# jonassibbesen/rpvg

Measured on AMD Instinct MI355X. Metric: read-pairs quantified/sec, higher is better.
Workload: dtype f64

## Files before the change

### include/rpvg_hip.h

```cpp
#ifndef RPVG_HIP_H
#define RPVG_HIP_H

#include <stdint.h>

#include "rpvg_batch.h"
#include "rpvg_rows.h"
#include "rpvg_index.h"
#include "rpvg_table.h"
#include "rpvg_samples.h"

#ifdef __cplusplus
extern "C" {
#endif

typedef enum rpvg_hip_status {
    RPVG_HIP_OK = 0,
    RPVG_HIP_ERR_NO_DEVICE = -1,
    RPVG_HIP_ERR_RUNTIME = -2,
    RPVG_HIP_ERR_INVALID = -3,
    RPVG_HIP_ERR_ALLOC = -4,
    RPVG_HIP_ERR_UNSUPPORTED = -5
} rpvg_hip_status;

typedef struct rpvg_hip_ctx rpvg_hip_ctx;
// ... 302 lines not shown
void rpvg_hip_gibbs_samples_free(rpvg_hip_ctx * ctx, rpvg_hip_gibbs_samples * samples);
int rpvg_hip_gibbs_table_build_resident(rpvg_hip_ctx * ctx, const rpvg_hip_gibbs_samples * samples, const rpvg_hip_em_problems * problems,
                                        uint32_t num_clusters, const uint64_t * cluster_path_off, const double * total_count,
                                        uint32_t num_gibbs_samples, rpvg_hip_gibbs_table ** table_out);

#define RPVG_HIP_COMM_ID_BYTES 128
int rpvg_hip_comm_unique_id(uint8_t * id_out);
int rpvg_hip_comm_init(rpvg_hip_ctx * ctx, const uint8_t * id, int world_size, int rank);
int rpvg_hip_comm_destroy(rpvg_hip_ctx * ctx);
int rpvg_hip_comm_init_all(rpvg_hip_ctx * const * ctxs, int num_contexts);
int rpvg_hip_comm_allreduce_sum_f64(rpvg_hip_ctx * ctx, double * device_buf, uint64_t n);
int rpvg_hip_gather(rpvg_hip_ctx * ctx, const double * local_values, uint64_t local_count, const uint64_t * counts, double * all_values);

int rpvg_hip_synth_dense_cluster(rpvg_hip_ctx * ctx, uint64_t seed, uint64_t num_rows, uint32_t num_paths,
                                 double * device_matrix, uint64_t ld, double * device_counts);
int rpvg_hip_synth_dense_rows(rpvg_hip_ctx * ctx, uint64_t seed, uint64_t row_begin, uint64_t num_rows, uint32_t num_paths,
                              double * device_matrix, uint64_t ld, double * device_counts);

int rpvg_hip_synth_dense_cluster_batch(rpvg_hip_ctx * ctx, uint64_t seed, uint64_t num_rows, uint32_t num_paths,
                                       rpvg_hip_batch ** batch_out);

int rpvg_hip_debug_log(rpvg_hip_ctx * ctx, uint64_t n, const double * x, double * out, int32_t use_table);

#define RPVG_HIP_EM_KERNELS 12
typedef struct rpvg_hip_em_kernel_stats {
    double ms;
    uint64_t launches;
    uint64_t problems;
    uint64_t iterations;
    uint64_t max_iterations;
    double alg_bytes;
} rpvg_hip_em_kernel_stats;
const char * rpvg_hip_em_kernel_name(int index);

typedef struct rpvg_hip_kernel_stats {
    double em_sparse_ms;      uint64_t em_sparse_launches;   double em_sparse_alg_bytes;
    double em_dense_ms;       uint64_t em_dense_launches;    double em_dense_alg_bytes;
    double loglik_ms;         uint64_t loglik_launches;      double loglik_evals;
    double build_ms;          uint64_t build_launches;
    double h2d_ms;            double h2d_bytes;
    uint64_t em_iterations_total;
    double search_pairs_possible; double search_pairs_table; double search_pairs_kept;
    rpvg_hip_em_kernel_stats em_kernel[RPVG_HIP_EM_KERNELS];
    double collapse_ms;
    double busy_ms;
    double gibbs_ms;
    double search_tile_ms;    uint64_t search_tile_launches;
    uint64_t gibbs_calls_completed;
    uint64_t gibbs_count_grid_problems;
    uint64_t gibbs_count_grid_iterations;
    uint64_t cover_grid_problems;
    uint64_t cover_grid_rounds;
    uint64_t nested_full_calls;
    uint64_t nested_full_sets;
    uint64_t nested_full_retained;
} rpvg_hip_kernel_stats;

int rpvg_hip_stats_get(rpvg_hip_ctx * ctx, rpvg_hip_kernel_stats * stats_out);
int rpvg_hip_stats_reset(rpvg_hip_ctx * ctx);
int rpvg_hip_stats_intervals(rpvg_hip_ctx * ctx, uint64_t capacity, double * start_ms, double * stop_ms, int32_t * family,
                             uint64_t * count_out);

#ifdef __cplusplus
}
#endif

// ... 2 lines not shown
```

### rpvg_amd/csrc/common.hpp

```cpp
#ifndef RPVG_HIP_COMMON_HPP
#define RPVG_HIP_COMMON_HPP

#include <hip/hip_runtime.h>

#include <algorithm>
#include <chrono>
#include <cstdarg>
#include <cstdint>
#include <cstdio>
#include <cstdlib>
#include <cstring>
#include <memory>
#include <mutex>
#include <new>
#include <string>
#include <functional>
#include <vector>

#include "../../include/rpvg_hip.h"
#include "search_plan.hpp"
#include "em_plan.hpp"
#include "batch_forms.hpp"

namespace rpvg_hip_detail {
// ... 771 lines not shown
    DeviceBuffer<uint32_t> d_prow_off, d_pent_col, d_bucket, d_order, d_seg_rows, d_seg_entries;
    DeviceBuffer<double> d_prow_count, d_prow_noise, d_pent_val, d_zero, d_wide_vectors, d_seg_zero, d_seg_total;
    DeviceBuffer<unsigned long long> d_wide_off;
    DeviceBuffer<unsigned char> d_queues;
    unsigned char * zeroed_queues = nullptr;
    std::shared_ptr<void> collapse;
    DeviceBuffer<double> fused_matrix[kEmMaxFusedDense];
    EmFusedDense fused[kEmMaxFusedDense];
    uint32_t num_fused = 0;
    hipEvent_t filled = nullptr, collapsed = nullptr, collapse_sorted = nullptr;
    EmProblemsView view(const EmProblemList & list, const EmOutputs & out) const {
        EmProblemsView v;
        v.col_off = list.d_col_off;
        v.row_base = list.d_row_base;
        v.ent_base = list.d_ent_base;
        v.kept_rows = out.d_kept_rows;
        v.zero_mass = d_zero.ptr;
        v.total_mass = out.d_total;
        v.prow_off = d_prow_off.ptr;
        v.prow_count = d_prow_count.ptr;
        v.prow_noise = d_prow_noise.ptr;
        v.pent_col = d_pent_col.ptr;
        v.pent_val = d_pent_val.ptr;
        return v;
    }
    ~EmSolveWork() {
        if (filled) (void) hipEventDestroy(filled);
        if (collapsed) (void) hipEventDestroy(collapsed);
        if (collapse_sorted) (void) hipEventDestroy(collapse_sorted);
    }
};
size_t emQueuesBytes();
uint32_t emFillSegmentRows();

struct EmGridControl {
    uint32_t done;
    uint32_t iterations;
    uint32_t conv_its;
    uint32_t viol;
    uint32_t error;
    uint32_t arrived;
};

struct EmGridProblem {
    uint32_t problem, columns;
    uint32_t rows, entries;
    uint32_t merged, pad;
    uint64_t row_base, ent_base, col_begin;
    double total_mass, zero_mass;
};

struct EmGridStorage {
    EmProblemsView problems;
    double * abundances;
    double * noise_count;
    uint32_t * iterations;
    const EmFusedDense * fused = nullptr;
    uint32_t num_fused = 0;
};

uint64_t emGridMinWork();
uint64_t gibbsGridMinWork();
bool emGridDenseRoute(uint32_t columns, uint32_t rows, uint32_t entries);
int runEmGridProblems(rpvg_hip_ctx * ctx, hipStream_t st, const EmGridProblem * problems, uint32_t count, const EmGridStorage & storage,
                      uint32_t max_em_its, double max_rel_em_conv);

// ... 115 lines not shown
```

### rpvg_amd/csrc/em_plan.hpp

```cpp
#ifndef RPVG_EM_PLAN_HPP
#define RPVG_EM_PLAN_HPP

#include <algorithm>
#include <cstddef>
#include <cstdint>

#ifndef RPVG_PLAN_FN
#if defined(__HIPCC__)
#define RPVG_PLAN_FN __host__ __device__ inline
#else
#define RPVG_PLAN_FN inline
#endif
#endif

namespace rpvg_em {

constexpr int kEmBins = 12;
constexpr int kEmGridBin = 11;
constexpr int kEmWideBin = 10;
constexpr int kEmWorkBuckets = 32;
constexpr uint32_t kEmMidGridMax = 8;
constexpr uint32_t kEmMidGridLog2 = 16;
constexpr uint32_t kEmMidBuckets = kEmWorkBuckets - kEmMidGridLog2;
constexpr int kEmStreamedBin = 3;
// ... 37 lines not shown

RPVG_PLAN_FN uint32_t emWorkBucket(const uint32_t rows, const uint32_t entries) {
    uint64_t work = static_cast<uint64_t>(entries) + rows + 1;
    uint32_t lg = 0;
    while (work > 1 && lg < static_cast<uint32_t>(kEmWorkBuckets - 1)) {
        work >>= 1;
        ++lg;
    }
    return static_cast<uint32_t>(kEmWorkBuckets - 1) - lg;
}

RPVG_PLAN_FN bool emIsMidSize(const uint32_t bin, const uint32_t bucket) { return bin == static_cast<uint32_t>(kEmStreamedBin) && bucket < kEmMidBuckets; }
RPVG_PLAN_FN bool emMidGridAllowed(const uint64_t grid_min_work) { return grid_min_work > (1ull << kEmMidGridLog2); }
RPVG_PLAN_FN bool emMidGridMoves(const bool allowed, const uint32_t mid) { return allowed && mid > 0 && mid <= kEmMidGridMax; }
RPVG_PLAN_FN int emRouteOf(const int bin, const uint32_t bucket, const bool moved) {
    return moved && emIsMidSize(static_cast<uint32_t>(bin), bucket) ? kEmGridBin : bin;
}

RPVG_PLAN_FN bool emIsRegisterBin(const int bin) { return bin == 4 || bin == 5 || bin == 6 || bin == 8 || bin == 9; }
RPVG_PLAN_FN int emStatsSlot(const int bin, const bool one_register_launch) {
    return emIsRegisterBin(bin) && one_register_launch ? static_cast<int>(kRegisterKernelIndex) : bin;
}

constexpr int kEmMaxFusedDense = 4;
constexpr uint32_t kEmDenseMaxCols = 2048;
RPVG_PLAN_FN bool emDenseRule(const uint32_t columns, const uint32_t rows, const uint32_t entries) {
    if (columns > kEmDenseMaxCols || columns < 2) return false;
    const uint64_t ld = (static_cast<uint64_t>(columns) + 1) & ~1ull;
    return 8ull * rows * ld <= 12ull * entries + 20ull * rows;
}

constexpr uint32_t kLdsMapPaths = 16384;
constexpr uint32_t kFillSegmentRows = 1024;
constexpr uint64_t kFillLongRowEntries = 32;
constexpr size_t kFillLongRowLds = kFillSegmentRows * (3 * sizeof(uint32_t) + sizeof(double));
constexpr size_t kFillDenseLds = kFillSegmentRows * 2 * sizeof(uint32_t);
constexpr uint64_t kFillLongRowMinWork = 1ull << 18;
RPVG_PLAN_FN size_t emFillDenseLdsBytes(const uint32_t lds_map_paths, const uint64_t widest_ld) {
    return lds_map_paths * sizeof(int32_t) + kFillDenseLds + 4 * static_cast<size_t>(widest_ld) * sizeof(double);
}

struct EmSolveKnobs {
    EmBinRule rule = {1u, 0, 1ull << 18};
    bool no_collapse = false;
    bool no_fused_dense = false;
    bool register_copies = true;
    bool one_register_launch = true;
    bool merged_launches = false;
    bool fill_thread_rows = false;
    double grid_scale = 1.0;
    bool few_streams = false;
    bool launch_early = false;
    bool wait_sort_only = false;
    bool join_on_stream = false;
    bool collapse_debug = false;
    bool has_bound_bytes = false;
    uint64_t bound_bytes = 0;
};

RPVG_PLAN_FN bool emStorageByBound(const uint64_t rows_bound, const uint64_t entries_bound, const uint64_t budget) {
    return rows_bound * 20 + entries_bound * 12 <= budget;
}
template <typename Count>
inline void emStorageBases(const Count * rows, const Count * entries, const uint32_t P, uint64_t * row_base, uint64_t * ent_base, uint64_t * rows_total,
                           uint64_t * entries_total) {
    uint64_t r = 0, e = 0;
    for (uint32_t p = 0; p < P; ++p) {
        row_base[p] = r;
        ent_base[p] = e;
        r += rows[p];
        e += entries[p];
    }
    *rows_total = r;
    *entries_total = e;
}

constexpr size_t kGibbsOneWorkgroupLdsLimit = 160 * 1024;
RPVG_PLAN_FN size_t gibbsOneWorkgroupLds(const uint32_t columns) {
    return (sizeof(double) * (2 * static_cast<size_t>(columns) + 256 / 64 + 2) + 15) & ~static_cast<size_t>(15);
}
RPVG_PLAN_FN bool gibbsTakesGrid(const uint32_t columns, const uint32_t rows, const uint32_t entries, const uint64_t grid_min_work) {
    const bool too_wide = gibbsOneWorkgroupLds(columns) > kGibbsOneWorkgroupLdsLimit;
    const bool too_large = grid_min_work != 0 && static_cast<uint64_t>(rows) + entries >= grid_min_work;
    return too_wide || too_large;
}
RPVG_PLAN_FN bool gibbsGridPossible(const uint32_t max_cols, const uint64_t max_cluster_work, const uint64_t grid_min_work) {
    return gibbsOneWorkgroupLds(max_cols) > kGibbsOneWorkgroupLdsLimit || (grid_min_work != 0 && max_cluster_work >= grid_min_work);
}

struct EmSolveShape {
    uint32_t P = 0, items_bound = 0, max_cols = 0, max_cluster_paths = 0;
    uint64_t max_cluster_work = 0, rows_capacity = 0;
    unsigned long long wide_capacity = 0;
    uint32_t cus = 0;
    int side_streams = 6;
    int hardware_queues = 4;
    bool collapse_wanted = false;
};
constexpr int kEmSideStreams = 6;
constexpr uint32_t kEmCollapseMaxProblems = (1u << 20) - 2;
constexpr uint64_t kEmCollapseMaxRows = 0x7fffffffull;

struct EmFillPlan {
    uint32_t fill_grid = 0;
    uint32_t dense_grid = 0;
    uint32_t lds_map_paths = 0;
    bool long_row_scratch = false;
    size_t fill_lds = 0;
};
inline EmFillPlan planEmFill(const EmSolveShape & s, const EmSolveKnobs & knobs) {
    EmFillPlan f;
    f.fill_grid = std::min<uint32_t>(s.items_bound, s.cus * 8);
    f.dense_grid = std::min<uint32_t>(s.items_bound, s.cus * 4);
    f.lds_map_paths = (std::min<uint32_t>(s.max_cluster_paths, kLdsMapPaths) + 3) & ~3u;
    f.long_row_scratch = !knobs.fill_thread_rows && s.max_cluster_work >= kFillLongRowMinWork;
    f.fill_lds = f.lds_map_paths * sizeof(int32_t) + (f.long_row_scratch ? kFillLongRowLds : 0);
    return f;
}

enum class EmVariant : uint8_t {
    kSparse64Resident, kSparse256Resident, kSparse1024Resident, kSparse256Streamed, kSparse1024Streamed, kSparseWide,
    kRegisterBins,
    kRegister1x16, kRegister2x16, kRegister4x16, kRegister1x32, kRegister2x32,
    kWaveBins,
    kSparse1024Bins
};
constexpr int kEmMainStream = -1;
struct EmLaunch {
    uint32_t bin;
    EmVariant variant;
    uint32_t grid;
    size_t lds;
    int stream;
};
inline bool operator==(const EmLaunch & a, const EmLaunch & b) {
    return a.bin == b.bin && a.variant == b.variant && a.grid == b.grid && a.lds == b.lds && a.stream == b.stream;
}
constexpr int kEmMaxLaunches = 11;

constexpr uint32_t kEmMaxRoles = 6;
struct EmRoles {
    uint32_t variants = 0;
    uint32_t grid = 0;
    uint32_t bin[kEmMaxRoles] = {};
};

struct EmSolvePlan {
    EmFillPlan fill;
    bool collapse = false;
// ... 96 lines not shown
```

### rpvg_amd/csrc/em_sparse.hip

```cpp

#include "common.hpp"

#include "collapse_plan.hpp"
#include "em_block.hpp"

#include <algorithm>
#include <memory>
#include <numeric>

using namespace rpvg_hip_detail;

namespace {

constexpr double kMinEmAbundance = 1e-8;
constexpr uint32_t kMinEmConvIts = 10;
static_assert(kEmBins == RPVG_HIP_EM_KERNELS, "a statistics slot per size bin (em_plan.hpp)");

struct EmQueues {
    uint32_t histogram[kEmBins * kEmWorkBuckets];
    uint32_t bucket_cursor[kEmBins * kEmWorkBuckets];
    uint32_t bin_start[kEmBins];
    uint32_t bin_count[kEmBins];
    uint32_t bin_cursor[kEmBins];
    uint32_t pad;
    unsigned long long wide_cursor;
    unsigned long long wide_overflow;
};


struct FillArgs {
    uint32_t num_problems;
    const uint32_t * num_problems_dev;
    uint32_t num_items;
    const uint32_t * num_items_dev;
    const uint64_t * seg_first;
    const uint32_t * item_problem;
    const uint32_t * prob_cluster;
    const uint32_t * col_path;
    const uint64_t * cluster_row_off;
    const uint64_t * cluster_path_off;
    const uint64_t * row_ent_off;
    const uint32_t * ent_path;
    const double * ent_prob;
    const double * row_count;
    const double * row_noise;
    EmProblemsView problems;
    uint32_t * seg_rows;
    uint32_t * seg_entries;
    double * seg_zero_mass;
    double * seg_total_mass;
    uint32_t * kept_entries;
    uint32_t * prob_bucket;
    EmQueues * queues;
    EmBinRule rule;
    uint32_t lds_map_paths;
    uint32_t long_row_scratch;
    uint32_t num_fused;
    EmFusedDense fused[kEmMaxFusedDense];
};

__device__ inline bool fillLongRows(const FillArgs & args, const uint32_t k) {
    const uint64_t c0 = args.cluster_row_off[k], c1 = args.cluster_row_off[k + 1];
    return args.long_row_scratch && args.row_ent_off[c1] - args.row_ent_off[c0] >= kFillLongRowEntries * (c1 - c0);
}

template <bool WRITE>
__global__ __launch_bounds__(256) void fillSegmentsKernel(const FillArgs args) {
    constexpr int BLOCK = 256;
    extern __shared__ __attribute__((aligned(16))) int32_t lds_map[];
    __shared__ uint32_t scratch[2 * (BLOCK / 64)];
    __shared__ double dscratch[BLOCK / 64];
    const uint32_t num_items = args.num_items_dev ? *args.num_items_dev : args.num_items;
    uint32_t mapped_problem = UINT32_MAX;
    for (uint32_t item = blockIdx.x; item < num_items; item += gridDim.x) {
        const uint32_t p = args.item_problem[item];
        if (WRITE) {
            bool fused = false;
            for (uint32_t f = 0; f < args.num_fused; ++f) fused = fused || args.fused[f].problem == p;
            if (fused) continue;
        }
        const uint32_t segment = static_cast<uint32_t>(item - args.seg_first[p]);
        const uint32_t k = args.prob_cluster[p];
        const uint32_t n_paths = static_cast<uint32_t>(args.cluster_path_off[k + 1] - args.cluster_path_off[k]);
        const uint32_t * cols = args.col_path + args.problems.col_off[p];
        const uint32_t n_cols = args.problems.paths(p);
        const bool use_map = n_paths <= args.lds_map_paths;
        const bool identity = n_cols == n_paths;
        __syncthreads();
        if (use_map && !identity && mapped_problem != p) {
            for (uint32_t i = threadIdx.x; i < n_paths; i += BLOCK) lds_map[i] = -1;
            __syncthreads();
            for (uint32_t c = threadIdx.x; c < n_cols; c += BLOCK) lds_map[cols[c]] = static_cast<int32_t>(c);
            __syncthreads();
            mapped_problem = p;
        }
        auto column_of = [&](const uint32_t path) -> int32_t {
            if (identity) return static_cast<int32_t>(path);
            if (use_map) return lds_map[path];
            uint32_t lo = 0, hi = n_cols;
            while (lo < hi) {
                const uint32_t mid = (lo + hi) >> 1;
                if (cols[mid] < path) lo = mid + 1;
                else hi = mid;
            }
            return (lo < n_cols && cols[lo] == path) ? static_cast<int32_t>(lo) : -1;
        };
        const uint64_t c0 = args.cluster_row_off[k], c1 = args.cluster_row_off[k + 1];
        const uint64_t r0 = c0 + static_cast<uint64_t>(segment) * kFillSegmentRows, r1 = min(c1, r0 + kFillSegmentRows);
        EmProblemsView::Slots at = {};
        if (WRITE) at = args.problems.slots(p);
        uint32_t * off = args.problems.prow_off + at.off;
        uint32_t run_rows = WRITE ? args.seg_rows[item] : 0, run_ent = WRITE ? args.seg_entries[item] : 0;
        double z = 0, t = 0;
        if (fillLongRows(args, k)) {
            uint32_t * row_n = reinterpret_cast<uint32_t *>(lds_map + args.lds_map_paths);
            uint32_t * row_slot = row_n + kFillSegmentRows, * row_eoff = row_slot + kFillSegmentRows;
            double * row_sum = reinterpret_cast<double *>(row_eoff + kFillSegmentRows);
            const uint32_t lane = threadIdx.x & 63, wave = threadIdx.x >> 6;
            const uint32_t seg_n = static_cast<uint32_t>(r1 - r0);
            for (uint32_t i = wave; i < seg_n; i += BLOCK / 64) {
                const uint64_t r = r0 + i;
                const uint64_t e0 = args.row_ent_off[r], e1 = args.row_ent_off[r + 1];
                uint32_t n = 0;
                double sum = 0;
                if (identity) {
                    n = static_cast<uint32_t>(e1 - e0);
                    if (WRITE) {
                        for (uint64_t e = e0 + lane; e < e1; e += 64) sum += args.ent_prob[e];
                    }
                } else {
                    for (uint64_t e = e0 + lane; e < e1; e += 64) {
                        if (column_of(args.ent_path[e]) >= 0) {
                            ++n;
                            sum += args.ent_prob[e];
                        }
                    }
                    for (int d = 32; d >= 1; d >>= 1) n += __shfl_xor(n, d, 64);
                }
                if (WRITE) sum = waveSumF64(sum);
                if (lane == 0) {
                    row_n[i] = n;
                    if (WRITE) row_sum[i] = sum;
                    if (!WRITE) {
                        const double c = args.row_count[r];
                        t += c;
                        if (!n) z += c;
                    }
// ... 28 lines not shown
                    const double nz = args.row_noise[r];
                    if (lane == 0) {
                        off[my_row] = my_ent;
                        args.problems.prow_count[at.row + my_row] = args.row_count[r];
                        args.problems.prow_noise[at.row + my_row] = nz;
                    }
                    const double keep = 1 - nz, rowsum = row_sum[i];
                    const uint64_t e0 = args.row_ent_off[r], e1 = args.row_ent_off[r + 1];
                    uint32_t base = 0;
                    for (uint64_t eb0 = e0; eb0 < e1; eb0 += 64) {
                        const uint64_t e = eb0 + lane;
                        const int32_t c = e < e1 ? column_of(args.ent_path[e]) : -1;
                        const unsigned long long kept = __ballot(c >= 0);
                        if (c >= 0) {
                            const uint32_t to = my_ent + base + static_cast<uint32_t>(__popcll(kept & ((1ull << lane) - 1)));
                            args.problems.pent_col[at.ent + to] = static_cast<uint32_t>(c);
                            args.problems.pent_val[at.ent + to] = (args.ent_prob[e] / rowsum) * keep;
                        }
                        base += static_cast<uint32_t>(__popcll(kept));
                    }
                }
            } else {
                z = blockReduceSum<double, BLOCK>(z, dscratch);
                t = blockReduceSum<double, BLOCK>(t, dscratch);
                if (threadIdx.x == 0) {
                    args.seg_rows[item] = tot_rows;
                    args.seg_entries[item] = tot_ent;
                    args.seg_zero_mass[item] = z;
                    args.seg_total_mass[item] = t;
                }
            }
            continue;
        }
        for (uint64_t rc = r0; rc < r1; rc += BLOCK) {
            const uint64_t r = rc + threadIdx.x;
            uint32_t n = 0;
            double rowsum = 0;
            uint64_t e0 = 0, e1 = 0;
            if (r < r1) {
                e0 = args.row_ent_off[r];
                e1 = args.row_ent_off[r + 1];
                for (uint64_t e = e0; e < e1; ++e) {
                    if (column_of(args.ent_path[e]) >= 0) {
                        ++n;
                        rowsum += args.ent_prob[e];
                    }
                }
                if (!WRITE) {
                    const double c = args.row_count[r];
                    t += c;
                    if (!n) z += c;
                }
            }
            uint32_t slot = n ? 1u : 0u, epos = n, tot_rows, tot_ent;
            blockExclusiveScanPair<BLOCK>(slot, epos, tot_rows, tot_ent, scratch);
            if (WRITE && n) {
                const uint32_t my_row = run_rows + slot;
                uint32_t my_ent = run_ent + epos;
                off[my_row] = my_ent;
                const double nz = args.row_noise[r];
                args.problems.prow_count[at.row + my_row] = args.row_count[r];
                args.problems.prow_noise[at.row + my_row] = nz;
                const double keep = 1 - nz;
                for (uint64_t e = e0; e < e1; ++e) {
                    const int32_t c = column_of(args.ent_path[e]);
                    if (c >= 0) {
                        args.problems.pent_col[at.ent + my_ent] = static_cast<uint32_t>(c);
                        args.problems.pent_val[at.ent + my_ent] = (args.ent_prob[e] / rowsum) * keep;
                        ++my_ent;
                    }
                }
            }
            run_rows += tot_rows;
            run_ent += tot_ent;
        }
        if (!WRITE) {
            z = blockReduceSum<double, BLOCK>(z, dscratch);
            t = blockReduceSum<double, BLOCK>(t, dscratch);
            if (threadIdx.x == 0) {
                args.seg_rows[item] = run_rows;
                args.seg_entries[item] = run_ent;
                args.seg_zero_mass[item] = z;
                args.seg_total_mass[item] = t;
            }
        }
    }
}

template <bool WRITE>
hipError_t launchFillSegments(const FillArgs & fa, const EmFillPlan & plan, hipStream_t st) {
    if (plan.fill_lds > kLdsOptIn) {
        const hipError_t e = hipFuncSetAttribute(reinterpret_cast<const void *>(&fillSegmentsKernel<WRITE>), hipFuncAttributeMaxDynamicSharedMemorySize, static_cast<int>(plan.fill_lds));
        if (e != hipSuccess) return e;
    }
    fillSegmentsKernel<WRITE><<<dim3(plan.fill_grid), dim3(256), plan.fill_lds, st>>>(fa);
    return hipSuccess;
}

constexpr int kDenseRowCache = 32;

__global__ __launch_bounds__(256) void fillDenseRowsKernel(const FillArgs args) {
    constexpr int BLOCK = 256;
// ... 687 lines not shown
    const uint32_t role = blockIdx.x % roles.variants, block = blockIdx.x / roles.variants;
    args.bin = roleBin(roles, role);
    switch (args.bin) {
        case 6: emRegisterBin<4, 16>(args, block, reg_lds); break;
        case 4: emRegisterBin<1, 16>(args, block, reg_lds); break;
        case 5: emRegisterBin<2, 16>(args, block, reg_lds); break;
        case 8: emRegisterBin<1, 32>(args, block, reg_lds); break;
        case 9: emRegisterBin<2, 32>(args, block, reg_lds); break;
        case kWaveSparseBin: emSparseBin<64, true>(args, block, reinterpret_cast<unsigned char *>(reg_lds), nullptr); break;
        default: break;
    }
}

template <int RPL, int COLS>
hipError_t launchEmRegister(const EmLaunchArgs & args, uint32_t grid, size_t lds, hipStream_t stream) {
    if (grid == 0) return hipSuccess;
    emRegisterBinKernel<RPL, COLS><<<dim3(grid), dim3(64), lds, stream>>>(args);
    return hipGetLastError();
}

hipError_t launchEmRegisterBins(const EmLaunchArgs & args, const EmRoles & roles, const size_t lds, hipStream_t stream) {
    const uint32_t grid = roles.variants * roles.grid;
    if (grid == 0) return hipSuccess;
    emRegisterKernel<<<dim3(grid), dim3(64), lds, stream>>>(args, roles);
    return hipGetLastError();
}

}

namespace rpvg_hip_detail {

size_t emQueuesBytes() { return sizeof(EmQueues); }
uint32_t emFillSegmentRows() { return kFillSegmentRows; }

EmSolveKnobs emSolveKnobs() {
    static const EmSolveKnobs once = []() {
        EmSolveKnobs k;
        k.rule.use_register_kernel = RPVG_EXPERIMENT_ENV("RPVG_HIP_NO_REGISTER_EM") == nullptr ? 1u : 0u;
        k.rule.streamed_small_work = RPVG_EXPERIMENT_ENV("RPVG_HIP_EM_STREAM_SMALL") ? std::strtoull(RPVG_EXPERIMENT_ENV("RPVG_HIP_EM_STREAM_SMALL"), nullptr, 10) : 0;
        k.no_collapse = RPVG_EXPERIMENT_ENV("RPVG_HIP_NO_EM_COLLAPSE") != nullptr;
        const char * launches = std::getenv("RPVG_HIP_EM_REGISTER_LAUNCHES");
        k.one_register_launch = !(launches && std::atoi(launches) == 5);
        k.fill_thread_rows = RPVG_EXPERIMENT_ENV("RPVG_HIP_FILL_THREAD_ROWS") != nullptr;
        k.grid_scale = RPVG_EXPERIMENT_ENV("RPVG_HIP_EM_GRID_SCALE") ? std::atof(RPVG_EXPERIMENT_ENV("RPVG_HIP_EM_GRID_SCALE")) : 1.0;
        k.few_streams = RPVG_EXPERIMENT_ENV("RPVG_HIP_EM_FEW_STREAMS") != nullptr;
        k.launch_early = RPVG_EXPERIMENT_ENV("RPVG_HIP_EM_LAUNCH_EARLY") != nullptr;
        k.wait_sort_only = RPVG_EXPERIMENT_ENV("RPVG_HIP_EM_WAIT_SORT_ONLY") != nullptr;
        k.join_on_stream = RPVG_EXPERIMENT_ENV("RPVG_HIP_EM_JOIN_ON_STREAM") != nullptr;
        k.collapse_debug = RPVG_EXPERIMENT_ENV("RPVG_HIP_EM_COLLAPSE_DEBUG") != nullptr;
        return k;
    }();
    EmSolveKnobs k = once;
    k.rule.grid_min_work = emGridMinWork();
    k.no_collapse = k.no_collapse || RPVG_EXPERIMENT_ENV("RPVG_HIP_NO_COLLAPSE") != nullptr;
    k.no_fused_dense = std::getenv("RPVG_HIP_NO_FUSED_DENSE") != nullptr;
    const char * separate = std::getenv("RPVG_HIP_EM_SEPARATE_LAUNCHES");
    k.merged_launches = !(separate && std::atoi(separate) != 0);
    const char * copies = std::getenv("RPVG_HIP_EM_COPIES");
    k.register_copies = copies ? std::atoi(copies) != 0 : true;
    const char * budget = std::getenv("RPVG_HIP_EM_BOUND_BYTES");
    k.has_bound_bytes = budget != nullptr;
    k.bound_bytes = budget ? static_cast<uint64_t>(std::atof(budget)) : 0;
    return k;
}

EmSolveShape emSolveShape(const rpvg_hip_ctx * ctx, const EmProblemList & list, const bool collapse_wanted) {
    EmSolveShape s;
    s.P = list.P_bound;
    s.items_bound = list.items_bound;
    s.max_cols = list.max_cols;
    s.max_cluster_paths = list.max_cluster_paths;
    s.max_cluster_work = list.max_cluster_work;
    s.rows_capacity = list.rows_capacity;
    s.wide_capacity = list.wide_capacity;
    s.cus = static_cast<uint32_t>(ctx->props.multiProcessorCount);
    s.side_streams = ctx->aux_count;
    s.hardware_queues = hardwareQueues();
    s.collapse_wanted = collapse_wanted;
    return s;
}

}

namespace {

static_assert(kEmSideStreams == rpvg_hip_ctx::kAuxStreams && kEmCollapseMaxProblems + 2 == kCollapseMaxMatrices, "em_plan.hpp restates these");

struct EmCountBuffers {
    DeviceBuffer<uint32_t> * seg_rows, * seg_entries;
    DeviceBuffer<double> * seg_zero, * seg_total;
// ... 3 lines not shown
                 const EmCountBuffers & buffers, const EmBinRule rule, EmQueues * queues, uint32_t * prob_bucket, const EmFillPlan & plan, FillArgs & fa) {
    hipStream_t st = ctx->stream;
    RPVG_HIP_CHECK(buffers.seg_rows->alloc(list.items_bound));
    RPVG_HIP_CHECK(buffers.seg_entries->alloc(list.items_bound));
    RPVG_HIP_CHECK(buffers.seg_zero->alloc(list.items_bound));
    RPVG_HIP_CHECK(buffers.seg_total->alloc(list.items_bound));
    fa = FillArgs{};
    fa.num_problems = list.P_bound;
    fa.num_problems_dev = list.d_num_problems;
    fa.num_items = list.items_bound;
    fa.num_items_dev = list.d_num_items;
    fa.seg_first = list.d_seg_first;
    fa.item_problem = list.d_item_problem;
    fa.prob_cluster = list.d_cluster;
    fa.col_path = list.d_col_path;
    fa.cluster_row_off = batch->cluster_row_off.ptr;
    fa.cluster_path_off = batch->cluster_path_off.ptr;
    fa.row_ent_off = batch->row_ent_off.ptr;
    fa.ent_path = batch->ent_path.ptr;
    fa.ent_prob = batch->ent_prob.ptr;
    fa.row_count = batch->row_count.ptr;
    fa.row_noise = batch->row_noise.ptr;
    fa.problems = view;
    fa.seg_rows = buffers.seg_rows->ptr;
    fa.seg_entries = buffers.seg_entries->ptr;
    fa.seg_zero_mass = buffers.seg_zero->ptr;
    fa.seg_total_mass = buffers.seg_total->ptr;
    fa.kept_entries = out.d_kept_entries;
    fa.prob_bucket = prob_bucket;
    fa.queues = queues;
    fa.rule = rule;
    fa.lds_map_paths = plan.lds_map_paths;
    fa.long_row_scratch = plan.long_row_scratch ? 1u : 0u;
    fa.num_fused = 0;
    RPVG_HIP_CHECK(launchFillSegments<false>(fa, plan, st));
    fillOffsetsKernel<<<dim3((list.P_bound + 255) / 256), dim3(256), 0, st>>>(fa);
    return RPVG_HIP_OK;
}

int lookForFusedDense(rpvg_hip_ctx * ctx, const uint32_t P, EmSolveWork & work, FillArgs & fa) {
    hipStream_t st = ctx->stream;
    DeviceBuffer<DenseCandidates> d_candidates;
    DenseCandidates * h_candidates = nullptr;
    RPVG_HIP_CHECK(d_candidates.alloc(1));
    if (pinnedAlloc(reinterpret_cast<void **>(&h_candidates), sizeof(DenseCandidates)) != hipSuccess) {
        setError("rpvg_hip_em_solve: out of page-locked host memory");
        return RPVG_HIP_ERR_ALLOC;
    }
    struct PinnedGuard {
        void * p;
        ~PinnedGuard() { pinnedFree(p); }
    } pinned_guard{h_candidates};
    RPVG_HIP_CHECK(zeroAsync(d_candidates.ptr, sizeof(DenseCandidates), st));
    denseCandidatesKernel<<<dim3((P + 255) / 256), dim3(256), 0, st>>>(fa, d_candidates.ptr);
    RPVG_HIP_CHECK(hipGetLastError());
    RPVG_HIP_CHECK(hipMemcpyAsync(h_candidates, d_candidates.ptr, sizeof(DenseCandidates), hipMemcpyDeviceToHost, st));
    {
        HostScope wait_scope("em_solve: the counts of the large problems");
        RPVG_HIP_CHECK(waitStream(st));
    }
    const uint32_t n = std::min<uint32_t>(h_candidates->count, kEmMaxFusedDense);
    for (uint32_t i = 0; i < n; ++i) {
        const DenseCandidate & c = h_candidates->list[i];
        if (!emGridDenseRoute(c.columns, c.rows, c.entries)) continue;
        const uint64_t ld = (static_cast<uint64_t>(c.columns) + 1) & ~1ull;
        DeviceBuffer<double> & m = work.fused_matrix[work.num_fused];
// ... 386 lines not shown
    ctx->spanEnd(span);
    ctx->stats.h2d_bytes += static_cast<double>(P * 4 + (P + 1) * 24 + ps.n_cols_total * 4);
    list.d_cluster = ps.d_cluster.ptr;
    list.d_col_off = ps.d_col_off.ptr;
    list.d_col_path = ps.d_col_path.ptr;
    list.d_seg_first = ps.d_seg_first.ptr;
    list.d_item_problem = ps.d_item_problem.ptr;
    if (!by_bound) {
        scope.reset(new HostScope("problems: counting pass"));
        EmSolveWork count_work;
        RPVG_HIP_CHECK(count_work.d_zero.alloc(P));
        const EmCountBuffers buffers{&count_work.d_seg_rows, &count_work.d_seg_entries, &count_work.d_seg_zero, &count_work.d_seg_total};
        FillArgs fa;
        const int rc = queueEmCount(ctx, batch, list, out, count_work.view(list, out), buffers, knobs.rule, nullptr, nullptr, planEmFill(emSolveShape(ctx, list, false), knobs), fa);
        if (rc != RPVG_HIP_OK) return rc;
        RPVG_HIP_CHECK(hipGetLastError());
        std::vector<uint32_t> kept_rows(P), kept_ent(P);
        RPVG_HIP_CHECK(hipMemcpyAsync(kept_rows.data(), out.d_kept_rows, P * sizeof(uint32_t), hipMemcpyDeviceToHost, st));
        RPVG_HIP_CHECK(hipMemcpyAsync(kept_ent.data(), out.d_kept_entries, P * sizeof(uint32_t), hipMemcpyDeviceToHost, st));
        RPVG_HIP_CHECK(waitStream(st));
        emStorageBases(kept_rows.data(), kept_ent.data(), P, row_base.data(), ent_base.data(), &rows_bound, &entries_bound);
        RPVG_HIP_CHECK(ps.d_row_base.upload(row_base.data(), P, st));
        RPVG_HIP_CHECK(ps.d_ent_base.upload(ent_base.data(), P, st));
    }
    list.d_row_base = ps.d_row_base.ptr;
    list.d_ent_base = ps.d_ent_base.ptr;
    list.rows_capacity = rows_bound;
    list.entries_capacity = entries_bound;
    return RPVG_HIP_OK;
}

}

extern "C" const char * rpvg_hip_em_kernel_name(int index) {
    static const char * const names[RPVG_HIP_EM_KERNELS] = {
        "emSparseKernel<64,true>", "emSparseKernel<256,true>", "emSparseKernel<256,false>", "emSparseKernel<1024,false>",
        "emRegisterBinKernel<1,16>", "emRegisterBinKernel<2,16>", "emRegisterBinKernel<4,16>", "emSparseKernel<1024,true>",
        "emRegisterBinKernel<1,32>", "emRegisterBinKernel<2,32>", "emSparseKernel<1024,false,WIDE>", "emGridAccumKernel"};
    if (index < 0 || index >= RPVG_HIP_EM_KERNELS) return nullptr;
    if (index == static_cast<int>(kRegisterKernelIndex) && emStatsSlot(static_cast<int>(kRegisterBins[0]), emSolveKnobs().one_register_launch) == index) return "emRegisterKernel";
    return names[index];
}

extern "C" int rpvg_hip_em_solve(rpvg_hip_ctx * ctx, const rpvg_hip_batch * batch, uint32_t max_em_its,
                                 double max_rel_em_conv, const rpvg_hip_em_problems * problems,
                                 rpvg_hip_em_results * results) {
    RPVG_REQUIRE(ctx && batch && problems && results, "rpvg_hip_em_solve: NULL argument");
    const uint32_t P = problems->num_problems;
    if (P == 0) return RPVG_HIP_OK;
    RPVG_REQUIRE(problems->cluster && problems->col_off && problems->col_path, "rpvg_hip_em_solve: NULL problem arrays");
    RPVG_REQUIRE(results->abundances && results->noise_count && results->total_count && results->iterations,
                 "rpvg_hip_em_solve: NULL result arrays");
    RPVG_REQUIRE(max_em_its > 0, "rpvg_hip_em_solve: max_em_its must be positive");

    std::lock_guard<std::mutex> lock(ctx->mutex);
    RPVG_HIP_CHECK(hipSetDevice(ctx->device));
    hipStream_t st = ctx->stream;

    std::vector<uint32_t> kept_rows(P), kept_ent(P);
    DeviceBuffer<uint32_t> d_iters, d_kept_rows, d_kept_ent;
    DeviceBuffer<double> d_abund, d_noise_count, d_total;
    DownloadPack outputs;
    outputs.add(d_abund, results->abundances, problems->col_off[P]);
    outputs.add(d_noise_count, results->noise_count, P);
    outputs.add(d_total, results->total_count, P);
    outputs.add(d_iters, results->iterations, P);
// ... 21 lines not shown
```

### rpvg_amd/hip.py

```python
from __future__ import annotations

import ctypes as C
import os
from typing import List, Optional, Sequence, Tuple

import numpy as np

from .batch import CClusterBatch, ClusterBatch

_HERE = os.path.dirname(os.path.abspath(__file__))
LIB_PATH = os.path.join(_HERE, "csrc", "librpvg_hip.so")

EXPORTS = [
    "rpvg_hip_device_count", "rpvg_hip_create", "rpvg_hip_create_uploader", "rpvg_hip_destroy", "rpvg_hip_last_error", "rpvg_hip_synchronize",
    "rpvg_hip_device_info", "rpvg_hip_malloc", "rpvg_hip_free", "rpvg_hip_memcpy_h2d", "rpvg_hip_memcpy_d2h",
    "rpvg_hip_batch_upload", "rpvg_hip_batch_free", "rpvg_hip_em_solve", "rpvg_hip_em_dense",
    "rpvg_hip_dense_from_cluster", "rpvg_hip_groups_build", "rpvg_hip_groups_free", "rpvg_hip_groups_collapse_info", "rpvg_hip_group_loglik",
    "rpvg_hip_synth_dense_cluster", "rpvg_hip_stats_get", "rpvg_hip_stats_reset", "rpvg_hip_stats_intervals", "rpvg_hip_em_kernel_name",
    "rpvg_hip_gibbs_read_counts", "rpvg_hip_min_path_cover", "rpvg_hip_min_path_cover_any", "rpvg_hip_cover_limits", "rpvg_hip_bounded_pair_posteriors", "rpvg_hip_pair_posteriors_get", "rpvg_hip_pair_posteriors_free",
    "rpvg_hip_em_dense_sharded", "rpvg_hip_synth_dense_rows", "rpvg_hip_synth_dense_cluster_batch", "rpvg_hip_comm_unique_id", "rpvg_hip_comm_init",
    "rpvg_hip_comm_destroy", "rpvg_hip_comm_allreduce_sum_f64", "rpvg_hip_comm_init_all", "rpvg_hip_gather", "rpvg_hip_host_register", "rpvg_hip_host_unregister", "rpvg_hip_group_conditionals",
    "rpvg_hip_group_gibbs", "rpvg_hip_group_gibbs_polyploid", "rpvg_hip_gibbs_sets_get", "rpvg_hip_gibbs_sets_free",
    "rpvg_hip_alignments_upload", "rpvg_hip_alignments_free", "rpvg_hip_read_rows_build", "rpvg_hip_read_rows_to_batch",
    "rpvg_hip_read_rows_view", "rpvg_hip_read_rows_sizes", "rpvg_hip_read_rows_free", "rpvg_hip_path_clusters", "rpvg_hip_debug_log",
    "rpvg_hip_nested_subset_em", "rpvg_hip_subset_em_get", "rpvg_hip_subset_em_free",
    "rpvg_hip_nested_full_subset_em", "rpvg_hip_subset_em_get_sets",
    "rpvg_hip_batch_cluster_totals", "rpvg_hip_batch_has_source_columns", "rpvg_hip_batch_source_columns_sizes",
    "rpvg_hip_batch_source_columns_get", "rpvg_hip_groups_build_from_sources", "rpvg_hip_groups_build_single_paths", "rpvg_hip_batch_upload_begin", "rpvg_hip_batch_upload_finish", "rpvg_hip_create_with_streams",
    "rpvg_hip_batch_upload_finish_queue", "rpvg_hip_batch_upload_finish_wait",
    "rpvg_hip_batch_upload_segments", "rpvg_hip_pinned_alloc", "rpvg_hip_pinned_free", "rpvg_hip_thread_wait_spin_us",
    "rpvg_hip_group_full_posteriors", "rpvg_hip_full_set_count",
    "rpvg_hip_frag_length_fit", "rpvg_hip_frag_length_table", "rpvg_hip_frag_length_table_get", "rpvg_hip_frag_length_table_free",
    "rpvg_hip_effective_lengths", "rpvg_hip_alignments_set_effective_lengths", "rpvg_hip_frag_length_eval",
    "rpvg_hip_align_index_create", "rpvg_hip_align_index_free", "rpvg_hip_align_index_add", "rpvg_hip_align_index_finish",
    "rpvg_hip_align_index_frag_counts", "rpvg_hip_align_index_view", "rpvg_hip_align_index_alignments",
    "rpvg_hip_path_table_upload", "rpvg_hip_path_table_free", "rpvg_hip_read_rows_to_batch_with_paths", "rpvg_hip_batch_path_group_ids",
    "rpvg_hip_name_groups_limits", "rpvg_hip_align_index_name_groups", "rpvg_hip_name_groups_view", "rpvg_hip_name_groups_free",
    "rpvg_hip_estimates_table_build", "rpvg_hip_estimates_table_tpm", "rpvg_hip_estimates_table_view", "rpvg_hip_estimates_table_limits",
    "rpvg_hip_estimates_table_free",
    "rpvg_hip_gibbs_table_build", "rpvg_hip_gibbs_table_view", "rpvg_hip_gibbs_table_rows", "rpvg_hip_gibbs_table_limits", "rpvg_hip_gibbs_table_free",
    "rpvg_hip_gibbs_read_counts_resident", "rpvg_hip_gibbs_samples_get", "rpvg_hip_gibbs_samples_free", "rpvg_hip_gibbs_table_build_resident",
    "rpvg_hip_align_index_alignments_collapsed",
    "rpvg_hip_batch_rows_sizes", "rpvg_hip_batch_rows_get",
    "rpvg_hip_segment_sort_words",
]

COMM_ID_BYTES = 128


class EngineError(RuntimeError):
    pass


class CEmProblems(C.Structure):
    _fields_ = [("num_problems", C.c_uint32), ("cluster", C.c_void_p), ("col_off", C.c_void_p), ("col_path", C.c_void_p),
                ("collapse_precision", C.c_double)]


class CEmResults(C.Structure):
    _fields_ = [("abundances", C.c_void_p), ("noise_count", C.c_void_p), ("total_count", C.c_void_p),
                ("iterations", C.c_void_p)]


class CGroupSpec(C.Structure):
    _fields_ = [("num_matrices", C.c_uint32), ("cluster", C.c_void_p), ("group_off", C.c_void_p),
                ("group_path_off", C.c_void_p), ("group_path", C.c_void_p), ("normalise", C.c_int32),
                ("collapse_precision", C.c_double)]


class CGibbsSpec(C.Structure):
    _fields_ = [("num_problems", C.c_uint32), ("group_size", C.c_uint32), ("matrix", C.c_void_p), ("num_chains", C.c_void_p),
                ("num_burn_its", C.c_void_p), ("num_gibbs_its", C.c_void_p), ("log_freq", C.c_void_p), ("num_generators", C.c_uint32),
                ("generator_problem_off", C.c_void_p), ("generator_problem", C.c_void_p), ("generator_words", C.c_void_p)]


class CGibbsSetsView(C.Structure):
    _fields_ = [("num_problems", C.c_uint32), ("group_size", C.c_uint32), ("set_off", C.POINTER(C.c_uint64)),
# ... 35 lines not shown
        ("h2d_ms", C.c_double), ("h2d_bytes", C.c_double),
        ("em_iterations_total", C.c_uint64),
        ("search_pairs_possible", C.c_double), ("search_pairs_table", C.c_double), ("search_pairs_kept", C.c_double),
        ("em_kernel", CEmKernelStats * EM_KERNELS),
        ("collapse_ms", C.c_double), ("busy_ms", C.c_double), ("gibbs_ms", C.c_double),
        ("search_tile_ms", C.c_double), ("search_tile_launches", C.c_uint64),
        ("gibbs_calls_completed", C.c_uint64),
        ("gibbs_count_grid_problems", C.c_uint64), ("gibbs_count_grid_iterations", C.c_uint64),
        ("cover_grid_problems", C.c_uint64), ("cover_grid_rounds", C.c_uint64),
        ("nested_full_calls", C.c_uint64), ("nested_full_sets", C.c_uint64), ("nested_full_retained", C.c_uint64),
    ]

    def as_dict(self):
        d = {n: getattr(self, n) for n, _ in self._fields_ if n != "em_kernel"}
        d["em_kernel"] = {em_kernel_name(i): {n: getattr(self.em_kernel[i], n) for n, _ in CEmKernelStats._fields_} for i in range(EM_KERNELS)}
        return d


GRID_NEVER = 2 ** 64 - 1


class CCoverLimits(C.Structure):
    _fields_ = [("workgroup_max_paths", C.c_uint32), ("chunk_rounds", C.c_uint32), ("default_grid_min_work", C.c_uint64),
                ("grid_max_rows", C.c_uint64), ("grid_max_entries", C.c_uint64), ("pick_block", C.c_uint32), ("pick_per_thread", C.c_uint32),
                ("pick_max_blocks", C.c_uint32), ("strike_block", C.c_uint32), ("strike_max_blocks", C.c_uint32), ("hist_max_paths", C.c_uint32)]


def cover_limits() -> CCoverLimits:
    out = CCoverLimits()
    lib().rpvg_hip_cover_limits(C.byref(out))
    return out


def em_kernel_name(index: int) -> str:
    f = lib().rpvg_hip_em_kernel_name
    f.restype = C.c_char_p
    return f(index).decode()


_lib = None


def lib() -> C.CDLL:
    global _lib
    if _lib is None:
        if not os.path.exists(LIB_PATH):
            raise EngineError(f"{LIB_PATH} is missing: build it with `python -c 'import __graft_entry__ as g; g.build()'` "
                              "(there is no CPU fallback)")
        L = C.CDLL(LIB_PATH)
        L.rpvg_hip_last_error.restype = C.c_char_p
        L.rpvg_hip_full_set_count.restype = C.c_uint64
        L.rpvg_hip_cover_limits.restype = None
        for name in EXPORTS:
            getattr(L, name)
        _lib = L
    return _lib


def _check(rc: int, what: str):
    if rc != 0:
        raise EngineError(f"{what} failed ({rc}): {lib().rpvg_hip_last_error().decode()}")


def device_count() -> int:
    n = C.c_int(0)
    rc = lib().rpvg_hip_device_count(C.byref(n))
    return n.value if rc == 0 else 0


class CClusterSegment(C.Structure):
    _fields_ = [("base", C.c_void_p), ("bytes", C.c_uint64), ("num_rows", C.c_uint32), ("num_groups", C.c_uint32), ("num_entries", C.c_uint32),
                ("num_paths", C.c_uint32), ("num_sources", C.c_uint32), ("has_paths", C.c_uint32), ("total_read_count", C.c_uint64),
                ("row_count_at", C.c_uint64), ("row_noise_at", C.c_uint64), ("row_grp_off_at", C.c_uint64), ("grp_idx_off_at", C.c_uint64),
                ("grp_prob_at", C.c_uint64), ("path_idx_at", C.c_uint64), ("path_group_id_at", C.c_uint64), ("path_source_off_at", C.c_uint64),
                ("source_id_at", C.c_uint64), ("has_columns", C.c_uint32), ("num_columns", C.c_uint32), ("num_column_paths", C.c_uint32),
                ("max_column_paths", C.c_uint32), ("col_count_at", C.c_uint64), ("col_end_at", C.c_uint64), ("col_path_at", C.c_uint64)]


class PinnedSegments:

    def __init__(self, host: ClusterBatch, with_paths: bool = True, columns=None):
        L = lib()
        L.rpvg_hip_pinned_free.argtypes = [C.c_void_p]
        K = host.num_clusters
        self.blocks = []
# ... 765 lines not shown
```

Measured before the change: 2.570 billion.

## Stage fill entries in LDS and write single-segment problems in one pass

The sparse EM fill kernel now cooperatively stages each row-block's entry paths and probabilities into LDS in coalesced pieces. Per-thread row walks then read from shared memory rather than strided global memory. Problems with a single segment are counted and written in the first pass, and the WRITE pass skips them. The LDS footprint grows, so the fill grid and launch bounds are cut to fewer workgroups per CU, and the old two-pass path stays reachable through an environment variable.

```diff
diff --git a/include/rpvg_hip.h b/include/rpvg_hip.h
--- a/include/rpvg_hip.h
+++ b/include/rpvg_hip.h
@@ -358,6 +358,13 @@
     double alg_bytes;
 } rpvg_hip_em_kernel_stats;
 const char * rpvg_hip_em_kernel_name(int index);
+typedef struct rpvg_em_fill_limits {
+    uint32_t segment_rows;
+    uint32_t stage_entries;
+    uint32_t lds_map_paths;
+    uint32_t block_rows;
+} rpvg_em_fill_limits;
+void rpvg_hip_em_fill_limits(rpvg_em_fill_limits * limits_out);
 
 typedef struct rpvg_hip_kernel_stats {
     double em_sparse_ms;      uint64_t em_sparse_launches;   double em_sparse_alg_bytes;
diff --git a/rpvg_amd/csrc/common.hpp b/rpvg_amd/csrc/common.hpp
--- a/rpvg_amd/csrc/common.hpp
+++ b/rpvg_amd/csrc/common.hpp
@@ -827,6 +827,7 @@
 };
 size_t emQueuesBytes();
 uint32_t emFillSegmentRows();
+uint32_t emFillStageEntries();
 
 struct EmGridControl {
     uint32_t done;
diff --git a/rpvg_amd/csrc/em_plan.hpp b/rpvg_amd/csrc/em_plan.hpp
--- a/rpvg_amd/csrc/em_plan.hpp
+++ b/rpvg_amd/csrc/em_plan.hpp
@@ -93,6 +93,11 @@
 
 constexpr uint32_t kLdsMapPaths = 16384;
 constexpr uint32_t kFillSegmentRows = 1024;
+constexpr uint32_t kFillStageEntries = 1536;
+constexpr size_t kFillBlockOffsetsLds = 258 * sizeof(uint64_t);
+RPVG_PLAN_FN size_t emFillStageLdsBytes(const uint32_t stage_entries) {
+    return stage_entries ? kFillBlockOffsetsLds + static_cast<size_t>(stage_entries) * (sizeof(double) + sizeof(int32_t)) : 0;
+}
 constexpr uint64_t kFillLongRowEntries = 32;
 constexpr size_t kFillLongRowLds = kFillSegmentRows * (3 * sizeof(uint32_t) + sizeof(double));
 constexpr size_t kFillDenseLds = kFillSegmentRows * 2 * sizeof(uint32_t);
@@ -109,6 +114,7 @@
     bool one_register_launch = true;
     bool merged_launches = false;
     bool fill_thread_rows = false;
+    uint32_t fill_stage_entries = 0;
     double grid_scale = 1.0;
     bool few_streams = false;
     bool launch_early = false;
@@ -167,15 +173,27 @@
     uint32_t dense_grid = 0;
     uint32_t lds_map_paths = 0;
     bool long_row_scratch = false;
+    uint32_t stage_entries = 0;
+    uint32_t workgroups_per_cu = 0;
     size_t fill_lds = 0;
 };
+constexpr size_t kCuLdsBytes = 160 * 1024;
+constexpr uint32_t kFillMaxWorkgroupsPerCu = 8;
+constexpr uint32_t kFillStagedWorkgroupsPerCu = 6;
+RPVG_PLAN_FN uint32_t emFillWorkgroupsPerCu(const size_t fill_lds) {
+    const size_t granules = (fill_lds + 64 + 511) / 512;
+    const size_t fit = kCuLdsBytes / (granules * 512);
+    return static_cast<uint32_t>(fit < 1 ? 1 : fit > kFillStagedWorkgroupsPerCu ? kFillStagedWorkgroupsPerCu : fit);
+}
 inline EmFillPlan planEmFill(const EmSolveShape & s, const EmSolveKnobs & knobs) {
     EmFillPlan f;
-    f.fill_grid = std::min<uint32_t>(s.items_bound, s.cus * 8);
     f.dense_grid = std::min<uint32_t>(s.items_bound, s.cus * 4);
     f.lds_map_paths = (std::min<uint32_t>(s.max_cluster_paths, kLdsMapPaths) + 3) & ~3u;
     f.long_row_scratch = !knobs.fill_thread_rows && s.max_cluster_work >= kFillLongRowMinWork;
-    f.fill_lds = f.lds_map_paths * sizeof(int32_t) + (f.long_row_scratch ? kFillLongRowLds : 0);
+    f.stage_entries = knobs.fill_stage_entries & ~3u;
+    f.fill_lds = f.lds_map_paths * sizeof(int32_t) + std::max<size_t>(f.long_row_scratch ? kFillLongRowLds : 0, emFillStageLdsBytes(f.stage_entries));
+    f.workgroups_per_cu = f.stage_entries ? emFillWorkgroupsPerCu(f.fill_lds) : kFillMaxWorkgroupsPerCu;
+    f.fill_grid = std::min<uint32_t>(s.items_bound, s.cus * f.workgroups_per_cu);
     return f;
 }
 
diff --git a/rpvg_amd/csrc/em_sparse.hip b/rpvg_amd/csrc/em_sparse.hip
--- a/rpvg_amd/csrc/em_sparse.hip
+++ b/rpvg_amd/csrc/em_sparse.hip
@@ -55,18 +55,21 @@
     EmBinRule rule;
     uint32_t lds_map_paths;
     uint32_t long_row_scratch;
+    uint32_t stage_entries;
     uint32_t num_fused;
     EmFusedDense fused[kEmMaxFusedDense];
 };
 
 __device__ inline bool fillLongRows(const FillArgs & args, const uint32_t k) {
+    if (!args.long_row_scratch) return false;
     const uint64_t c0 = args.cluster_row_off[k], c1 = args.cluster_row_off[k + 1];
-    return args.long_row_scratch && args.row_ent_off[c1] - args.row_ent_off[c0] >= kFillLongRowEntries * (c1 - c0);
+    return args.row_ent_off[c1] - args.row_ent_off[c0] >= kFillLongRowEntries * (c1 - c0);
 }
 
 template <bool WRITE>
-__global__ __launch_bounds__(256) void fillSegmentsKernel(const FillArgs args) {
+__global__ __launch_bounds__(256, kFillStagedWorkgroupsPerCu) void fillSegmentsKernel(const FillArgs args) {
     constexpr int BLOCK = 256;
+    constexpr int kStageTurn = 2;
     extern __shared__ __attribute__((aligned(16))) int32_t lds_map[];
     __shared__ uint32_t scratch[2 * (BLOCK / 64)];
     __shared__ double dscratch[BLOCK / 64];
@@ -81,6 +84,10 @@
         }
         const uint32_t segment = static_cast<uint32_t>(item - args.seg_first[p]);
         const uint32_t k = args.prob_cluster[p];
+        const bool long_rows = fillLongRows(args, k);
+        const bool one_pass = args.stage_entries && args.problems.prow_off && !long_rows && args.seg_first[p + 1] - args.seg_first[p] == 1;
+        if (WRITE && one_pass) continue;
+        const bool write = WRITE || one_pass;
         const uint32_t n_paths = static_cast<uint32_t>(args.cluster_path_off[k + 1] - args.cluster_path_off[k]);
         const uint32_t * cols = args.col_path + args.problems.col_off[p];
         const uint32_t n_cols = args.problems.paths(p);
@@ -108,11 +115,11 @@
         const uint64_t c0 = args.cluster_row_off[k], c1 = args.cluster_row_off[k + 1];
         const uint64_t r0 = c0 + static_cast<uint64_t>(segment) * kFillSegmentRows, r1 = min(c1, r0 + kFillSegmentRows);
         EmProblemsView::Slots at = {};
-        if (WRITE) at = args.problems.slots(p);
+        if (write) at = args.problems.slots(p);
         uint32_t * off = args.problems.prow_off + at.off;
         uint32_t run_rows = WRITE ? args.seg_rows[item] : 0, run_ent = WRITE ? args.seg_entries[item] : 0;
         double z = 0, t = 0;
-        if (fillLongRows(args, k)) {
+        if (long_rows) {
             uint32_t * row_n = reinterpret_cast<uint32_t *>(lds_map + args.lds_map_paths);
             uint32_t * row_slot = row_n + kFillSegmentRows, * row_eoff = row_slot + kFillSegmentRows;
             double * row_sum = reinterpret_cast<double *>(row_eoff + kFillSegmentRows);
@@ -207,42 +214,140 @@
             }
             continue;
         }
+        const uint32_t stage = args.stage_entries;
+        uint64_t * blk_off = reinterpret_cast<uint64_t *>(lds_map + args.lds_map_paths);
+        double * st_val = reinterpret_cast<double *>(reinterpret_cast<char *>(blk_off) + kFillBlockOffsetsLds);
+        int32_t * st_col = reinterpret_cast<int32_t *>(st_val + stage);
         for (uint64_t rc = r0; rc < r1; rc += BLOCK) {
             const uint64_t r = rc + threadIdx.x;
+            const uint32_t nb = static_cast<uint32_t>(min(static_cast<uint64_t>(BLOCK), r1 - rc));
             uint32_t n = 0;
             double rowsum = 0;
             uint64_t e0 = 0, e1 = 0;
+            double count = 0, nz = 0;
             if (r < r1) {
                 e0 = args.row_ent_off[r];
                 e1 = args.row_ent_off[r + 1];
+                count = args.row_count[r];
+                if (write) nz = args.row_noise[r];
+            }
+            const bool walks = r < r1 && (!stage || e1 - e0 > stage);
+            auto pieceEnd = [&](const uint32_t i0) -> uint32_t {
+                const uint64_t limit = blk_off[i0] + stage;
+                if (blk_off[nb] <= limit) return nb;
+                uint32_t lo = i0, hi = nb - 1;
+                while (lo < hi) {
+                    const uint32_t mid = (lo + hi + 1) >> 1;
+                    if (blk_off[mid] <= limit) lo = mid;
+                    else hi = mid - 1;
+                }
+                return lo;
+            };
+            uint32_t staged0 = 0, staged1 = 0;
+            auto stagePiece = [&](const uint32_t i0, const uint32_t i1) {
+                __syncthreads();
+                const uint64_t base = blk_off[i0];
+                const uint32_t len = static_cast<uint32_t>(blk_off[i1] - base);
+                for (uint32_t j0 = threadIdx.x; j0 < len; j0 += kStageTurn * BLOCK) {
+                    uint32_t path[kStageTurn];
+                    double val[kStageTurn];
+#pragma unroll
+                    for (int u = 0; u < kStageTurn; ++u) {
+                        const uint32_t j = j0 + u * BLOCK;
+                        path[u] = j < len ? args.ent_path[base + j] : 0u;
+                        val[u] = write && j < len ? args.ent_prob[base + j] : 0.0;
+                    }
+#pragma unroll
+                    for (int u = 0; u < kStageTurn; ++u) {
+                        const uint32_t j = j0 + u * BLOCK;
+                        if (j < len) {
+                            st_col[j] = column_of(path[u]);
+                            if (write) st_val[j] = val[u];
+                        }
+                    }
+                }
+                __syncthreads();
+                staged0 = i0;
+                staged1 = i1;
+            };
+            if (stage) {
+                __syncthreads();
+                if (r < r1) blk_off[threadIdx.x] = e0;
+                if (threadIdx.x + 1 == nb) blk_off[nb] = e1;
+                __syncthreads();
+                for (uint32_t i0 = 0; i0 < nb;) {
+                    const uint32_t i1 = pieceEnd(i0);
+                    if (i1 == i0) {
+                        ++i0;
+                        continue;
+                    }
+                    stagePiece(i0, i1);
+                    if (threadIdx.x >= i0 && threadIdx.x < i1) {
+                        const uint32_t j1 = static_cast<uint32_t>(e1 - blk_off[i0]);
+                        for (uint32_t j = static_cast<uint32_t>(e0 - blk_off[i0]); j < j1; ++j) {
+                            if (st_col[j] >= 0) {
+                                ++n;
+                                if (write) rowsum += st_val[j];
+                            }
+                        }
+                    }
+                    i0 = i1;
+                }
+            }
+            if (walks) {
                 for (uint64_t e = e0; e < e1; ++e) {
                     if (column_of(args.ent_path[e]) >= 0) {
                         ++n;
                         rowsum += args.ent_prob[e];
                     }
                 }
-                if (!WRITE) {
-                    const double c = args.row_count[r];
-                    t += c;
-                    if (!n) z += c;
-                }
+            }
+            if (!WRITE && r < r1) {
+                t += count;
+                if (!n) z += count;
             }
             uint32_t slot = n ? 1u : 0u, epos = n, tot_rows, tot_ent;
             blockExclusiveScanPair<BLOCK>(slot, epos, tot_rows, tot_ent, scratch);
-            if (WRITE && n) {
+            if (write) {
                 const uint32_t my_row = run_rows + slot;
                 uint32_t my_ent = run_ent + epos;
-                off[my_row] = my_ent;
-                const double nz = args.row_noise[r];
-                args.problems.prow_count[at.row + my_row] = args.row_count[r];
-                args.problems.prow_noise[at.row + my_row] = nz;
-                const double keep = 1 - nz;
-                for (uint64_t e = e0; e < e1; ++e) {
-                    const int32_t c = column_of(args.ent_path[e]);
-                    if (c >= 0) {
-                        args.problems.pent_col[at.ent + my_ent] = static_cast<uint32_t>(c);
-                        args.problems.pent_val[at.ent + my_ent] = (args.ent_prob[e] / rowsum) * keep;
-                        ++my_ent;
+                double keep = 0;
+                if (n) {
+                    off[my_row] = my_ent;
+                    args.problems.prow_count[at.row + my_row] = count;
+                    args.problems.prow_noise[at.row + my_row] = nz;
+                    keep = 1 - nz;
+                }
+                if (stage) {
+                    for (uint32_t i0 = 0; i0 < nb;) {
+                        const uint32_t i1 = pieceEnd(i0);
+                        if (i1 == i0) {
+                            ++i0;
+                            continue;
+                        }
+                        if (staged0 != i0 || staged1 != i1) stagePiece(i0, i1);
+                        if (n && threadIdx.x >= i0 && threadIdx.x < i1) {
+                            const uint32_t j1 = static_cast<uint32_t>(e1 - blk_off[i0]);
+                            for (uint32_t j = static_cast<uint32_t>(e0 - blk_off[i0]); j < j1; ++j) {
+                                const int32_t c = st_col[j];
+                                if (c >= 0) {
+                                    args.problems.pent_col[at.ent + my_ent] = static_cast<uint32_t>(c);
+                                    args.problems.pent_val[at.ent + my_ent] = (st_val[j] / rowsum) * keep;
+                                    ++my_ent;
+                                }
+                            }
+                        }
+                        i0 = i1;
+                    }
+                }
+                if (walks && n) {
+                    for (uint64_t e = e0; e < e1; ++e) {
+                        const int32_t c = column_of(args.ent_path[e]);
+                        if (c >= 0) {
+                            args.problems.pent_col[at.ent + my_ent] = static_cast<uint32_t>(c);
+                            args.problems.pent_val[at.ent + my_ent] = (args.ent_prob[e] / rowsum) * keep;
+                            ++my_ent;
+                        }
                     }
                 }
             }
@@ -996,6 +1101,7 @@
 
 size_t emQueuesBytes() { return sizeof(EmQueues); }
 uint32_t emFillSegmentRows() { return kFillSegmentRows; }
+uint32_t emFillStageEntries() { return kFillStageEntries; }
 
 EmSolveKnobs emSolveKnobs() {
     static const EmSolveKnobs once = []() {
@@ -1020,6 +1126,9 @@
     k.no_fused_dense = std::getenv("RPVG_HIP_NO_FUSED_DENSE") != nullptr;
     const char * separate = std::getenv("RPVG_HIP_EM_SEPARATE_LAUNCHES");
     k.merged_launches = !(separate && std::atoi(separate) != 0);
+    const char * two_pass = std::getenv("RPVG_HIP_EM_FILL_TWO_PASS");
+    k.fill_stage_entries = two_pass && std::atoi(two_pass) != 0 ? 0u : kFillStageEntries;
+    if (k.fill_stage_entries && RPVG_EXPERIMENT_ENV("RPVG_HIP_EM_FILL_STAGE")) k.fill_stage_entries = static_cast<uint32_t>(std::atoi(RPVG_EXPERIMENT_ENV("RPVG_HIP_EM_FILL_STAGE")));
     const char * copies = std::getenv("RPVG_HIP_EM_COPIES");
     k.register_copies = copies ? std::atoi(copies) != 0 : true;
     const char * budget = std::getenv("RPVG_HIP_EM_BOUND_BYTES");
@@ -1089,6 +1198,7 @@
     fa.rule = rule;
     fa.lds_map_paths = plan.lds_map_paths;
     fa.long_row_scratch = plan.long_row_scratch ? 1u : 0u;
+    fa.stage_entries = plan.stage_entries;
     fa.num_fused = 0;
     RPVG_HIP_CHECK(launchFillSegments<false>(fa, plan, st));
     fillOffsetsKernel<<<dim3((list.P_bound + 255) / 256), dim3(256), 0, st>>>(fa);
@@ -1541,6 +1651,14 @@
 
 }
 
+extern "C" void rpvg_hip_em_fill_limits(rpvg_em_fill_limits * limits_out) {
+    if (!limits_out) return;
+    limits_out->segment_rows = emFillSegmentRows();
+    limits_out->stage_entries = emFillStageEntries();
+    limits_out->lds_map_paths = kLdsMapPaths;
+    limits_out->block_rows = 256;
+}
+
 extern "C" const char * rpvg_hip_em_kernel_name(int index) {
     static const char * const names[RPVG_HIP_EM_KERNELS] = {
         "emSparseKernel<64,true>", "emSparseKernel<256,true>", "emSparseKernel<256,false>", "emSparseKernel<1024,false>",
diff --git a/rpvg_amd/hip.py b/rpvg_amd/hip.py
--- a/rpvg_amd/hip.py
+++ b/rpvg_amd/hip.py
@@ -42,7 +42,7 @@
     "rpvg_hip_gibbs_read_counts_resident", "rpvg_hip_gibbs_samples_get", "rpvg_hip_gibbs_samples_free", "rpvg_hip_gibbs_table_build_resident",
     "rpvg_hip_align_index_alignments_collapsed",
     "rpvg_hip_batch_rows_sizes", "rpvg_hip_batch_rows_get",
-    "rpvg_hip_segment_sort_words",
+    "rpvg_hip_segment_sort_words", "rpvg_hip_em_fill_limits",
 ]
 
 COMM_ID_BYTES = 128
@@ -144,6 +144,16 @@
     return out
 
 
+class CEmFillLimits(C.Structure):
+    _fields_ = [("segment_rows", C.c_uint32), ("stage_entries", C.c_uint32), ("lds_map_paths", C.c_uint32), ("block_rows", C.c_uint32)]
+
+
+def em_fill_limits() -> CEmFillLimits:
+    out = CEmFillLimits()
+    lib().rpvg_hip_em_fill_limits(C.byref(out))
+    return out
+
+
 def em_kernel_name(index: int) -> str:
     f = lib().rpvg_hip_em_kernel_name
     f.restype = C.c_char_p
@@ -163,6 +173,7 @@
         L.rpvg_hip_last_error.restype = C.c_char_p
         L.rpvg_hip_full_set_count.restype = C.c_uint64
         L.rpvg_hip_cover_limits.restype = None
+        L.rpvg_hip_em_fill_limits.restype = None
         for name in EXPORTS:
             getattr(L, name)
         _lib = L
```

Measured after the change: 2.503 billion. 0.974x the previous value.
